# SeoYeonnLee/Video-Chapter-Generation

Hardware: AMD Instinct MI355X
Metric: clip-windows/sec (16f×224²+128tok) train-step at 1/2/4/8 MI355X; % HBM roofline (higher is better)
Workload: dtype bf16; 1 GPU; TwoStream train step: TSM-ResNet-50 + BERT-base + ChapterHead(mlp), B=64 windows/GPU of 16x224^2 frames + 128 tokens, fused clip+AdamW; global_batch=64, seq_len=128, frames=16, resolution=224, text_fill=n_valid ~ U[L/2, L], parallelism=dp1

## Files before the change

### video-chapter-generation_amd/csrc/igemm_fast.hip

```cpp
#include "fastload.h"

namespace vcg {

typedef __attribute__((address_space(3))) char lds_char;
__device__ __forceinline__ uint32_t lds_u32(const void* p) { return (uint32_t)(uintptr_t)(const lds_char*)p; }

template <int BN> __device__ __forceinline__ int st_slot(int row, int chunk) {
  if constexpr (BN == 128) return chunk ^ (row & 15);
  else return chunk ^ ((row >> 1) & 7);
}

template <int BM, int BN>
__device__ __forceinline__ void stage_put(bf16_t* stA, bf16_t* stB, int wm, int wn, int lane, int i, int j,
                                          const float (&v)[4]) {
  const int g = lane >> 4, ci = lane & 15;
  const int trow = (wm & 1) * 64 + i * 16 + ci;
  const int tcol = wn * (BN / 2) + j * 16 + 4 * g;
  bf16_t* reg = (BN == 128 && trow >= 64) ? stB : stA;
  const int row = BN == 128 ? (trow & 63) : trow;
  const uint32_t addr = lds_u32(reg + row * BN + 8 * st_slot<BN>(row, tcol >> 3) + (tcol & 7));
  uint2 q;
  q.x = (uint32_t)f2bf(v[0]) | ((uint32_t)f2bf(v[1]) << 16);
  q.y = (uint32_t)f2bf(v[2]) | ((uint32_t)f2bf(v[3]) << 16);
  asm volatile("ds_write_b64 %0, %1" ::"v"(addr), "v"(q) : "memory");
// ... 1161 lines not shown
    if (i < steps) issue_next(i);
  int kt = 0, tile = 0, cur = 0;
  for (int s = 0; s < steps; ++s) {
    const int ahead = min(STAGES - 1, steps - 1 - s);
    if (s + STAGES - 1 < steps) issue_next(cur == 0 ? STAGES - 1 : cur - 1);
    if (STAGES == 3 && ahead >= 2) __builtin_amdgcn_s_waitcnt(waitcnt_vm(2 * NLD));
    else if (ahead >= 1) __builtin_amdgcn_s_waitcnt(waitcnt_vm(NLD));
    else __builtin_amdgcn_s_waitcnt(waitcnt_vm(0));
    __builtin_amdgcn_s_barrier();
    if (kt == 0) FAST_STAMP(tile, 0);
    const bf16_t* Ac = As + cur * AE;
    const bf16_t* Bc = Bs + cur * BE;
#pragma unroll
    for (int s2 = 0; s2 < 2; ++s2) {
      s16x8 af[MT], bfr[NT];
#pragma unroll
      for (int i = 0; i < MT; ++i) af[i] = fast_frag(Ac, wm * 64 + i * 16, lane, s2);
#pragma unroll
      for (int j = 0; j < NT; ++j) bfr[j] = fast_frag(Bc, wn * (BN / 2) + j * 16, lane, s2);
#pragma unroll
      for (int i = 0; i < MT; ++i)
#pragma unroll
        for (int j = 0; j < NT; ++j)
          acc[i][j] = __builtin_amdgcn_mfma_f32_16x16x32_bf16(bfr[j], af[i], acc[i][j], 0, 0, 0);
    }
    __builtin_amdgcn_s_waitcnt(0xC07F);
    __builtin_amdgcn_s_barrier();
    if (++kt == ntiles) {
      FAST_STAMP(tile, 1);
      const int mt = by + tile * gy;
      bf16_t* stA = As + cur * AE;
      bf16_t* stB = BM == 256 ? stA + 64 * BN : Bs + cur * BE;
      const bool staged = true;
      if constexpr (BWD) {
#pragma unroll
        for (int h = 0; h < BM / 128; ++h) {
          if ((wm >> 1) == h) {
#pragma unroll
            for (int j = 0; j < NT; ++j)
#pragma unroll
              for (int i = 0; i < MT; ++i) {
                float v[4] = {acc[i][j][0], acc[i][j][1], acc[i][j][2], acc[i][j][3]};
                if constexpr (AM == OP_DENSE_K2) {
#pragma unroll
                  for (int r = 0; r < 4; ++r) v[r] += bv[j][r];
                }
                stage_put<BM, BN>(stA, stB, wm, wn, lane, i, j, v);
              }
          }
          FAST_STAMP(tile, 2);
          stage_flush_bwd<BM, BN, EPI == EPI_BWD_AFF>(stA, stB, p, Cout, mt * BM + 128 * h, n0, cpar, b1, b2, b3, p.M);
        }
      } else if constexpr (EPI == EPI_STATS) {
#pragma unroll
        for (int h = 0; h < BM / 128; ++h) {
          if ((wm >> 1) == h) {
#pragma unroll
            for (int j = 0; j < NT; ++j)
#pragma unroll
              for (int i = 0; i < MT; ++i) {
                float v[4] = {acc[i][j][0], acc[i][j][1], acc[i][j][2], acc[i][j][3]};
                stage_put<BM, BN>(stA, stB, wm, wn, lane, i, j, v);
              }
          }
          stage_flush_stats<BM, BN>(stA, stB, p, Cout, mt * BM + 128 * h, n0, scnt, b1, b2, b3, p.M);
        }
      } else if constexpr (EPI == EPI_STORE_AUX) {
        if constexpr (BM == 128) epilogue_staged_aux<BM, BN>(acc, p, bv, Cout, stA, stB, mt * BM, n0, wm, wn, lane);
      } else if (BM == 256 || (staged && !RES && p.aux == nullptr && (p.ldc & 7) == 0 &&
                               ((uintptr_t)p.C & 15) == 0)) {
        epilogue_staged<BM, BN>(acc, p, bv, Cout, stA, stB, mt * BM, n0, wm, wn, lane, p.M);
      } else if (RES && (staged || p.obits) && p.aux == nullptr &&
                 (RES == 2 ? (staged && !p.res_sc) : (p.res_round && p.act == ACT_RELU)) &&
                 ((p.ldc | p.ldr | p.N) & 7) == 0 && (((uintptr_t)p.residual | (uintptr_t)p.C) & 15) == 0) {
        if constexpr (BM == 128 && RES)
          epilogue_staged_res<BM, BN, RES == 2>(acc, p, bv, Cout, Res, stA, stB, mt * BM, n0, wm, wn, lane, p.M);
      } else {
        if constexpr (BM == 128)
          gemm_epilogue<bf16_t, BM, BN, EPI>(acc, p, red, bv, Cout, Res, mt * BM, n0, wm, wn, lane, mt, mtiles);
      }
      FAST_STAMP(tile, 3);
#pragma unroll
      for (int i = 0; i < MT; ++i)
#pragma unroll
        for (int j = 0; j < NT; ++j) acc[i][j] = f32x4{0.f, 0.f, 0.f, 0.f};
      kt = 0;
      ++tile;
    }
    cur = cur == STAGES - 1 ? 0 : cur + 1;
  }
  if constexpr (EPI == EPI_STATS)
    stats_finish<BM, BN>(p, reinterpret_cast<float*>(smem), scnt, b1, b2, b3, n0, by, bx, gy, (p.M + 127) / 128);
  if constexpr (BWD) {
    if (p.bwd.nred > 0) bwd_finish<BM, BN>(p, reinterpret_cast<float*>(smem), cpar + 4 * BN, b1, b2, b3, n0, by);
  }
}

template <int BM, int BN, int AM, int EPI, int RES, int XF = 0>
__global__ __launch_bounds__(BM * 2) __attribute__((amdgpu_waves_per_eu(EPI == EPI_BWD_AFF && BN == 64 ? 3 : 2)))
void igemm_fast_kernel(GemmParams p) {
  if constexpr (EPI == EPI_BWD_STREAM && BN == 128)
    bwd_stream128_body<XF>(p);
  else if constexpr (EPI == EPI_BWD_STREAM)
    bwd_stream_body<AM, XF>(p);
  else
    igemm_fast_body<BM, BN, AM, EPI, RES>(p);
}

static int grid_rows(int M, int N, int z, int BM, int BN, int epi) {
  const int nx = (N + BN - 1) / BN, mtiles = (M + BM - 1) / BM;
  const int resident = (BM == 256 ? 1 : (BN == 128 || epi == EPI_BWD ? 2 : 3)) * 256;
  int gy = resident / (nx * z);
  if (gy >= 8) gy &= ~7;
  if (gy > mtiles) gy = mtiles >= 8 ? (mtiles & ~7) : mtiles;
  if (gy < 1) gy = 1;
  return gy;
}

static int fast_bn_cols(int N) { return (N % 128 == 0 || N > 64 * 3) ? 128 : 64; }

static int fast_bm(int, int, int, bool) { return 128; }

int fast_grid_rows(int M, int N, int z, int epi) {
  return grid_rows(M, N, z, fast_bm(M, N, z, false), fast_bn_cols(N), epi);
}

static bool bwd_light(const GemmParams& p) {
  const BwdEpi& e = p.bwd;
  return !e.res && !e.bits && !e.y2 && e.tsm_T == 0;
}


constexpr int PATCH_MAXPIX = 256;
constexpr int PATCH_SLICES = PATCH_MAXPIX / 8;
constexpr int PATCH_RING = 3;

struct PatchGeom {
  int R, TM, TPI, PW, NP, NS;
  unsigned long long* stamps;
};
#define PATCH_STAMP(k)                                                                        \
  do {                                                                                        \
    if (g.stamps && blockIdx.x == 0 && threadIdx.x == 0 && lt < 64) g.stamps[lt * 6 + (k)] = __builtin_amdgcn_s_memtime(); \
  } while (0)

__device__ __forceinline__ int pswz(int pix, int c) { return (c + (pix & ~1)) & 7; }

__device__ __forceinline__ s16x8 patch_frag(const bf16_t* P, int pix, int lane, int s2) {
  return *reinterpret_cast<const s16x8*>(P + pix * 64 + 8 * pswz(pix, 4 * s2 + (lane >> 4)));
}

typedef __attribute__((address_space(3))) const char patch_lds_t;

template <int EPI, bool DG, int PW>
__global__ __launch_bounds__(256) __attribute__((amdgpu_waves_per_eu(1, 1)))
void conv3x3_patch_kernel(GemmParams p, PatchGeom g) {
  static_assert(PW == 32 || PW == 64, "patch row pitch");
  constexpr int BM = 128, BN = 64, NW = 4, MT = 4, NT = 2;
  constexpr int PE = PATCH_SLICES * 512;
  constexpr int YE = 128 * 64;
  constexpr bool BWD = EPI == EPI_BWD_AFF;
  constexpr int NY = BWD ? PATCH_RING : 0;
  constexpr int NIP = 8 + (BWD ? 4 : 0);
  __shared__ __attribute__((aligned(1024))) char smem[(PATCH_RING * PE + NY * YE) * 2];
  bf16_t* Ps = reinterpret_cast<bf16_t*>(smem);
  bf16_t* Ys = Ps + PATCH_RING * PE;

  const int tid = threadIdx.x, lane = tid & 63, wave = __builtin_amdgcn_readfirstlane(tid >> 6);
  const int wm = wave >> 1, wn = wave & 1;
  const int nx = p.N / BN, gy = gridDim.x / nx;
  int bx, by;
  if ((gy & 7) == 0) {
    const int sidx = blockIdx.x >> 3;
    bx = sidx % nx;
    by = (sidx / nx) * 8 + (blockIdx.x & 7);
  } else {
    bx = blockIdx.x % nx;
    by = blockIdx.x / nx;
  }
  const int n0 = bx * BN;
  bf16_t* Cout = reinterpret_cast<bf16_t*>(p.C);
  const int mtiles = p.M / g.TM;
  const int my_tiles = by < mtiles ? (mtiles - 1 - by) / gy + 1 : 0;
  const BwdEpi& e = p.bwd;
  if (my_tiles == 0) {
    if (BWD && e.nred > 0 && tid < BN)
      for (int r = 0; r < e.nred; ++r) e.part[((long long)by * e.nred + r) * p.N + n0 + tid] = 0.f;
    return;
  }

  const OpArgs& a = p.a;
  const uint32_t nbytes = (uint32_t)min(a.bytes, (long long)0xFFFFFF00LL);
  const __amdgpu_buffer_rsrc_t rsrc =
      __builtin_amdgcn_make_buffer_rsrc(const_cast<void*>(a.ptr), 0, nbytes, 0x00020000);
  const uint32_t ybytes = (BWD && e.y) ? (uint32_t)min((long long)p.M * p.ldc * 2, (long long)0xFFFFFF00LL) : 0u;
  const __amdgpu_buffer_rsrc_t yrsrc =
      __builtin_amdgcn_make_buffer_rsrc(const_cast<void*>(BWD ? e.y : a.ptr), 0, ybytes, 0x00020000);
  const int HW = a.H * a.W;
  auto issue_piece = [&](int lt, int tg, int img, int h0, int q) {
    if (q < 8) {
      bf16_t* dst = Ps + (lt % PATCH_RING) * PE;
      const int slice = min(wave + NW * q, g.NS - 1);
      const int pix = 8 * slice + (lane >> 3);
      const int pr = pix / PW, pc = pix % PW;
      const int h = h0 - 1 + pr, w = pc - 1;
      const bool ok = pix < g.NP && (unsigned)h < (unsigned)a.H && (unsigned)w < (unsigned)a.W;
      const int csrc = ((lane & 7) - (pix & ~1)) & 7;
      const uint32_t voff = ok ? (uint32_t)((((img * HW + h * a.W + w) << 6) + 8 * csrc) * 2) : nbytes;
      __builtin_amdgcn_raw_ptr_buffer_load_lds(rsrc, (lds_void_t*)(dst + slice * 512), 16, voff, 0, 0, 0);
    } else if constexpr (BWD) {
      bf16_t* ydst = Ys + (lt % PATCH_RING) * YE;
      const int r0 = 32 * wave + 8 * (q - 8), r = r0 + (lane >> 3);
      const uint32_t voff =
          r < g.TM ? (uint32_t)(((long long)(tg * g.TM + r) * p.ldc + n0 + 8 * (lane & 7)) * 2) : ybytes;
      __builtin_amdgcn_raw_ptr_buffer_load_lds(yrsrc, (lds_void_t*)(ydst + r0 * 64), 16, ybytes ? voff : 0u, 0, 0, 0);
    }
  };
  auto issue_tile = [&](int lt) {
    const int tg = by + lt * gy, img = tg / g.TPI, h0 = (tg - img * g.TPI) * g.R;
#pragma unroll
    for (int q = 0; q < NIP; ++q) issue_piece(lt, tg, img, h0, q);
  };
  int rowpix[MT];
#pragma unroll
  for (int i = 0; i < MT; ++i) {
    const int ml = wm * 64 + i * 16 + (lane & 15);
    const int r = ml / a.W, w = ml - r * a.W;
    rowpix[i] = ml < g.TM ? r * PW + w : 0;
  }
  s16x8 breg[9][2][NT];
  {
    const bf16_t* B = reinterpret_cast<const bf16_t*>(p.b.ptr);
#pragma unroll
    for (int j = 0; j < NT; ++j) {
      const bf16_t* row = B + (long long)(n0 + wn * (BN / 2) + j * 16 + (lane & 15)) * p.b.ld + 8 * (lane >> 4);
#pragma unroll
      for (int t = 0; t < 9; ++t)
#pragma unroll
        for (int s2 = 0; s2 < 2; ++s2) breg[t][s2][j] = *reinterpret_cast<const s16x8*>(row + 64 * t + 32 * s2);
    }
  }
  constexpr int CPR = BN / 8, KC = 128 * BN / 8 / 256;
  const int cc = tid % CPR, ncol = n0 + 8 * cc;
  float mu[8], sc[8], sh[8];
#pragma unroll
  for (int i = 0; i < 8; ++i) {
    mu[i] = (BWD && e.mean) ? e.mean[ncol + i] : 0.f;
    sc[i] = (BWD && e.msc) ? e.msc[ncol + i] : 0.f;
    sh[i] = (BWD && e.msh) ? e.msh[ncol + i] : 0.f;
  }
  __builtin_amdgcn_s_waitcnt(waitcnt_vm(0));
  issue_tile(0);
  if (my_tiles > 1) issue_tile(1);

  const bool mask = BWD && e.msc != nullptr && e.y != nullptr;
  float b1[8], b2[8], b3[8];
  int scnt = 0;
#pragma unroll
  for (int i = 0; i < 8; ++i) b1[i] = b2[i] = b3[i] = 0.f;
  uint4 q[KC], yq[KC];
  int pm0 = 0, pmlim = 0;
  auto process = [&](int k) {
    const int m = pm0 + (tid + 256 * k) / CPR;
    if (m >= pmlim) return;
    uint4* dst = reinterpret_cast<uint4*>(Cout + (long long)m * p.ldc + ncol);
    if constexpr (EPI == EPI_STORE) {
      *dst = q[k];
    } else if constexpr (EPI == EPI_STATS) {
      *dst = q[k];
      float v[8];
      unpack8(q[k], v);
      if (scnt == 0) {
#pragma unroll
        for (int i = 0; i < 8; ++i) b1[i] = v[i];
      }
      ++scnt;
#pragma unroll
      for (int i = 0; i < 8; ++i) {
        const float d = v[i] - b1[i];
        b2[i] += d;
        b3[i] = fmaf(d, d, b3[i]);
      }
    } else {
      float v[8], yy[8];
      unpack8(q[k], v);
      unpack8(yq[k], yy);
      if (mask) {
#pragma unroll
        for (int i = 0; i < 8; ++i) v[i] = fmaf(yy[i], sc[i], sh[i]) > 0.f ? v[i] : 0.f;
      }
      uint4 o;
      o.x = (uint32_t)f2bf(v[0]) | ((uint32_t)f2bf(v[1]) << 16);
      o.y = (uint32_t)f2bf(v[2]) | ((uint32_t)f2bf(v[3]) << 16);
      o.z = (uint32_t)f2bf(v[4]) | ((uint32_t)f2bf(v[5]) << 16);
      o.w = (uint32_t)f2bf(v[6]) | ((uint32_t)f2bf(v[7]) << 16);
      *dst = o;
      if (e.nred > 0) {
        unpack8(o, v);
#pragma unroll
        for (int i = 0; i < 8; ++i) {
          b1[i] += v[i];
          b2[i] = fmaf(v[i], yy[i] - mu[i], b2[i]);
        }
      }
    }
  };

  for (int lt = 0; lt < my_tiles; ++lt) {
    PATCH_STAMP(0);
    if (lt + 1 < my_tiles) __builtin_amdgcn_s_waitcnt(waitcnt_vm(NIP));
    else __builtin_amdgcn_s_waitcnt(waitcnt_vm(0));
    __builtin_amdgcn_s_barrier();
    PATCH_STAMP(1);
    const bool pre = lt + 2 < my_tiles;
    const int tg2 = by + (lt + 2) * gy, img2 = tg2 / g.TPI, h02 = (tg2 - img2 * g.TPI) * g.R;
    const bool prev = lt > 0;
    PATCH_STAMP(2);
    const bf16_t* P = Ps + (lt % PATCH_RING) * PE;
    f32x4 acc[MT][NT];
#pragma unroll
    for (int i = 0; i < MT; ++i)
#pragma unroll
      for (int j = 0; j < NT; ++j) acc[i][j] = f32x4{0.f, 0.f, 0.f, 0.f};
    uint32_t fa[MT][3][2];
#pragma unroll
    for (int i = 0; i < MT; ++i)
#pragma unroll
      for (int c = 0; c < 3; ++c) {
        const int pix = rowpix[i] + c;
        const uint32_t a0 = lds_u32(P + pix * 64 + 8 * pswz(pix, lane >> 4));
        fa[i][c][0] = a0;
        fa[i][c][1] = a0 ^ 64u;
      }
    auto unit_reads = [&](s16x8 (&f)[MT], int u) {
      const int t = u >> 1, kh = t / 3, kw = t - 3 * (t / 3);
      const int rh = DG ? 2 - kh : kh, cw = DG ? 2 - kw : kw;
#pragma unroll
      for (int i = 0; i < MT; ++i)
        f[i] = *reinterpret_cast<const __attribute__((address_space(3))) s16x8*>(
            (patch_lds_t*)(uintptr_t)fa[i][cw][u & 1] + rh * PW * 128);
    };
    s16x8 af[3][MT];
    unit_reads(af[0], 0);
    unit_reads(af[1], 1);
#pragma unroll
    for (int u = 0; u < 18; ++u) {
      if (u + 2 < 18) unit_reads(af[(u + 2) % 3], u + 2);
      if (u < NIP && pre) issue_piece(lt + 2, tg2, img2, h02, u);
      if constexpr (NIP + 2 * KC <= 18) {
        if (u >= NIP && ((u - NIP) & 1) == 0 && ((u - NIP) >> 1) < KC && prev) process((u - NIP) >> 1);
      } else {
        if (u >= 18 - KC && prev) process(u - (18 - KC));
      }
#pragma unroll
      for (int i = 0; i < MT; ++i)
#pragma unroll
        for (int j = 0; j < NT; ++j)
          acc[i][j] = __builtin_amdgcn_mfma_f32_16x16x32_bf16(breg[u >> 1][u & 1][j], af[u % 3][i], acc[i][j], 0, 0, 0);
      __builtin_amdgcn_sched_barrier(0);
    }
    PATCH_STAMP(3);
    __builtin_amdgcn_s_waitcnt(0xC07F);
    __builtin_amdgcn_s_barrier();
    PATCH_STAMP(4);
    bf16_t* stA = Ps + (lt % PATCH_RING) * PE;
#pragma unroll
    for (int j = 0; j < NT; ++j)
#pragma unroll
      for (int i = 0; i < MT; ++i) {
        float v[4] = {acc[i][j][0], acc[i][j][1], acc[i][j][2], acc[i][j][3]};
        stage_put<BM, BN>(stA, stA, wm, wn, lane, i, j, v);
      }
    asm volatile("s_waitcnt lgkmcnt(0)" ::: "memory");
    __builtin_amdgcn_s_barrier();
    const bf16_t* Y = Ys + (lt % PATCH_RING) * YE;
#pragma unroll
    for (int k = 0; k < KC; ++k) {
      const int trow = (tid + 256 * k) / CPR;
      asm volatile("ds_read_b128 %0, %1" : "=v"(q[k]) : "v"(lds_u32(stA + trow * BN + 8 * st_slot<BN>(trow, cc))) : "memory");
      if constexpr (BWD)
        asm volatile("ds_read_b128 %0, %1" : "=v"(yq[k]) : "v"(lds_u32(Y + trow * 64 + 8 * cc)) : "memory");
    }
    asm volatile("s_waitcnt lgkmcnt(0)" ::: "memory");
    pm0 = (by + lt * gy) * g.TM;
    pmlim = pm0 + g.TM;
    PATCH_STAMP(5);
  }
#pragma unroll
  for (int k = 0; k < KC; ++k) process(k);
  __builtin_amdgcn_s_waitcnt(waitcnt_vm(0));
  if constexpr (EPI == EPI_STATS)
    stats_finish<BM, BN>(p, reinterpret_cast<float*>(smem), scnt, b1, b2, b3, n0, by, bx, gy, (p.M + 127) / 128);
  if constexpr (BWD) {
    if (e.nred > 0) {
      float* inv = reinterpret_cast<float*>(smem) + 3 * 256 * 8;
      __syncthreads();
      if (tid < BN) inv[tid] = e.invstd ? e.invstd[n0 + tid] : 0.f;
      bwd_finish<BM, BN>(p, reinterpret_cast<float*>(smem), inv, b1, b2, b3, n0, by);
    }
  }
}

constexpr int SPATCH_MAXPIX = 1024;

struct StemGeom {
  int R, TM, TPI, PW, NP, NS, NR;
  unsigned long long* stamps;
};

template <int EPI>
__global__ __launch_bounds__(256) __attribute__((amdgpu_waves_per_eu(2, 2)))
void stem_patch_kernel(GemmParams p, StemGeom g) {
  constexpr int BM = 128, BN = 64, NW = 4, MT = 4, NT = 2, KHMAX = 8, RING = 3, NIP = 4;
  constexpr int PE = SPATCH_MAXPIX * 8;
  __shared__ __attribute__((aligned(1024))) char smem[RING * PE * 2];
  bf16_t* Ps = reinterpret_cast<bf16_t*>(smem);
  const int tid = threadIdx.x, lane = tid & 63, wave = __builtin_amdgcn_readfirstlane(tid >> 6);
  const int wm = wave >> 1, wn = wave & 1;
  const int nx = p.N / BN, gy = gridDim.x / nx;
  int bx, by;
  if ((gy & 7) == 0) {
    const int sidx = blockIdx.x >> 3;
    bx = sidx % nx;
    by = (sidx / nx) * 8 + (blockIdx.x & 7);
  } else {
    bx = blockIdx.x % nx;
    by = blockIdx.x / nx;
  }
  const int n0 = bx * BN;
  bf16_t* Cout = reinterpret_cast<bf16_t*>(p.C);
  const int mtiles = p.M / g.TM;
  const int my_tiles = by < mtiles ? (mtiles - 1 - by) / gy + 1 : 0;
  if (my_tiles == 0) return;

  const OpArgs& a = p.a;
  const int KH = a.KH;
  const uint32_t nbytes = (uint32_t)min(a.bytes, (long long)0xFFFFFF00LL);
  const __amdgpu_buffer_rsrc_t rsrc =
      __builtin_amdgcn_make_buffer_rsrc(const_cast<void*>(a.ptr), 0, nbytes, 0x00020000);
  auto issue_piece = [&](int lt, int img, int h0, int q) {
    bf16_t* dst = Ps + (lt % RING) * PE;
    const int slice = min(wave + NW * q, g.NS - 1);
    const int pix = 64 * slice + lane;
    const int pr = pix / g.PW, pc = pix - pr * g.PW;
    const int ih = 2 * h0 - a.pad + pr, sx = pc - a.pw;
    const bool ok = pix < g.NP && (unsigned)ih < (unsigned)a.H && (unsigned)sx < (unsigned)a.W;
    const uint32_t voff = ok ? (uint32_t)((((img * a.H + ih) * a.W + sx) << 3) * 2) : nbytes;
    __builtin_amdgcn_raw_ptr_buffer_load_lds(rsrc, (lds_void_t*)(dst + slice * 512), 16, voff, 0, 0, 0);
  };
  auto issue_tile = [&](int lt) {
    const int tg = by + lt * gy, img = tg / g.TPI, h0 = (tg - img * g.TPI) * g.R;
#pragma unroll
    for (int q = 0; q < NIP; ++q) issue_piece(lt, img, h0, q);
  };
  int rowpix[MT];
#pragma unroll
  for (int i = 0; i < MT; ++i) {
    const int ml = wm * 64 + i * 16 + (lane & 15);
    const int r = ml / a.GW, w = ml - r * a.GW;
    rowpix[i] = ml < g.TM ? 2 * r * g.PW + w : 0;
  }
  s16x8 breg[KHMAX][NT];
  {
    const bf16_t* B = reinterpret_cast<const bf16_t*>(p.b.ptr);
#pragma unroll
    for (int j = 0; j < NT; ++j) {
      const bf16_t* row = B + (long long)(n0 + wn * (BN / 2) + j * 16 + (lane & 15)) * p.b.ld + 8 * (lane >> 4);
#pragma unroll
      for (int kh = 0; kh < KHMAX; ++kh)
        breg[kh][j] = kh < KH ? *reinterpret_cast<const s16x8*>(row + 32 * kh) : s16x8{0, 0, 0, 0, 0, 0, 0, 0};
    }
  }
  constexpr int CPR = BN / 8, KC = 128 * BN / 8 / 256;
  const int cc = tid % CPR, ncol = n0 + 8 * cc;
  __builtin_amdgcn_s_waitcnt(waitcnt_vm(0));
  issue_tile(0);
  if (my_tiles > 1) issue_tile(1);

  float b1[8], b2[8], b3[8];
  int scnt = 0;
#pragma unroll
  for (int i = 0; i < 8; ++i) b1[i] = b2[i] = b3[i] = 0.f;
  uint4 q[KC];
  int pm0 = 0, pmlim = 0;
  auto process = [&](int k) {
    const int m = pm0 + (tid + 256 * k) / CPR;
    if (m >= pmlim) return;
    *reinterpret_cast<uint4*>(Cout + (long long)m * p.ldc + ncol) = q[k];
    if constexpr (EPI == EPI_STATS) {
      float v[8];
      unpack8(q[k], v);
      if (scnt == 0) {
#pragma unroll
        for (int i = 0; i < 8; ++i) b1[i] = v[i];
      }
      ++scnt;
#pragma unroll
      for (int i = 0; i < 8; ++i) {
        const float d = v[i] - b1[i];
        b2[i] += d;
        b3[i] = fmaf(d, d, b3[i]);
      }
    }
  };

  for (int lt = 0; lt < my_tiles; ++lt) {
    if (lt + 1 < my_tiles) __builtin_amdgcn_s_waitcnt(waitcnt_vm(NIP));
    else __builtin_amdgcn_s_waitcnt(waitcnt_vm(0));
    __builtin_amdgcn_s_barrier();
    const bool pre = lt + 2 < my_tiles;
    const int tg2 = by + (lt + 2) * gy, img2 = tg2 / g.TPI, h02 = (tg2 - img2 * g.TPI) * g.R;
    const bool prev = lt > 0;
    const bf16_t* P = Ps + (lt % RING) * PE;
#pragma unroll
    for (int i = 0; i < MT; ++i) asm volatile("" : "+v"(rowpix[i]));
    f32x4 acc[MT][NT];
#pragma unroll
    for (int i = 0; i < MT; ++i)
#pragma unroll
      for (int j = 0; j < NT; ++j) acc[i][j] = f32x4{0.f, 0.f, 0.f, 0.f};
    auto unit_reads = [&](s16x8 (&f)[MT], int kh) {
#pragma unroll
      for (int i = 0; i < MT; ++i)
        f[i] = *reinterpret_cast<const s16x8*>(P + (rowpix[i] + kh * g.PW + (lane >> 4)) * 8);
    };
    s16x8 af[3][MT];
    unit_reads(af[0], 0);
    unit_reads(af[1], 1);
#pragma unroll
    for (int u = 0; u < KHMAX; ++u) {
      if (u < KH) {
        if (u + 2 < KH) unit_reads(af[(u + 2) % 3], u + 2);
        if (u < NIP && pre) issue_piece(lt + 2, img2, h02, u);
        if (u >= 1 && u - 1 < KC && prev) process(u - 1);
#pragma unroll
        for (int i = 0; i < MT; ++i)
#pragma unroll
          for (int j = 0; j < NT; ++j)
            acc[i][j] = __builtin_amdgcn_mfma_f32_16x16x32_bf16(breg[u][j], af[u % 3][i], acc[i][j], 0, 0, 0);
        __builtin_amdgcn_sched_barrier(0);
      }
    }
    if (prev) {
// ... 49 lines not shown
  g.PW = p.a.GW + p.a.KW - 1;
  g.NR = 2 * R + p.a.KH - 2;
  g.NP = g.NR * g.PW;
  g.NS = (g.NP + 63) / 64;
  return g;
}

static int patch_pitch(int W) { return W + 2 <= 32 ? 32 : 64; }

static int patch_rows(const GemmParams& p, int amode) {
  const char* e = getenv("VCG_NO_PATCH");
  const bool off = e && e[0] == '1';
  const OpArgs& a = p.a;
  if (off || (amode != OP_IM2COL && amode != OP_DGRAD) || a.C != 64 || a.KH != 3 || a.KW != 3 || a.stride != 1 ||
      a.pad != 1 || a.tsm_fold != 0 || a.tKW != 0 || a.sw != 0 || a.GH != a.H || a.GW != a.W || p.N % 64 != 0 ||
      p.K != 9 * 64 || p.batch_inner > 0 || p.residual || p.aux || p.bias || p.act != ACT_NONE || a.W + 2 > 64 ||
      !bwd_light(p) || p.bwd.nred > 2)
    return 0;
  for (int R = min(a.H, 128 / a.W); R >= 1; --R)
    if (a.H % R == 0 && (R + 2) * patch_pitch(a.W) <= PATCH_MAXPIX) return R;
  return 0;
}

static PatchGeom patch_geom(const GemmParams& p, int R) {
  PatchGeom g{};
  g.R = R;
  g.TM = R * p.a.W;
  g.TPI = p.a.H / R;
  g.PW = patch_pitch(p.a.W);
  g.NP = (R + 2) * g.PW;
  g.NS = (g.NP + 7) / 8;
  return g;
}

static int patch_grid_rows(const GemmParams& p, const PatchGeom& g) {
  const int nx = p.N / 64, mtiles = p.M / g.TM;
  int gy = 256 / nx;
  gy = min(gy, min(mtiles, (p.M + 127) / 128));
  if (gy >= 8) gy &= ~7;
  return max(gy, 1);
}

static bool bwd_stream_ok(const GemmParams& p) {
  const char* v = getenv("VCG_BWD_STREAM");
  if (v && v[0] == '0') return false;
  const BwdEpi& e = p.bwd;
  const bool dense = p.a.KH == 0 && p.a.GH == 0;
  if (!dense || (p.K != 64 && p.K != 128 && p.K != 256) || p.N % 64 != 0 || p.batch_inner > 0 || p.ldc != p.N || p.a.ld != p.K ||
      !e.res || e.msc || e.sub || bwd_light(p))
    return false;
  if ((e.y && !e.bits) || (e.y2 && !e.y)) return false;
  if ((e.y || e.bits) && e.nred < 2) return false;
  if (e.tsm_T > 0 && e.tsm_fold % 32 != 0) return false;
  if (p.K == 256 && ((e.tsm_T > 0 && e.tsm_fold % 64 != 0) || e.y)) return false;
  if (p.K == 256 && ((uintptr_t)p.b.ptr & 15 || p.b.ld % 8 != 0)) return false;
  if (((uintptr_t)p.C | (uintptr_t)e.res | (uintptr_t)e.y | (uintptr_t)e.y2 | (uintptr_t)p.a.ptr) & 15) return false;
  if (e.res_s > 1 && (p.M % e.hw) != 0) return false;
  if (e.pj > 0) {
    if (e.y || !e.bits || e.pj != 64 || p.K > 128 || ((uintptr_t)e.a2 & 15) || !e.ppart) return false;
    if (((uintptr_t)p.b.ptr & 15) || p.b.ld % 8 != 0) return false;
  }
  return true;
}

static int bwd_stream_tn(const GemmParams& p) {
  const BwdEpi& e = p.bwd;
  const char* v = getenv("VCG_BWD_STREAM");
  if ((v && v[0] == '6') || p.bwd.pj > 0) return 64;
  return p.K == 256 && p.N % 128 == 0 && !e.y && (e.tsm_T <= 0 || e.tsm_fold % 128 == 0) ? 128 : 64;
}

static int bwd_stream_rows(const GemmParams& p) {
  const int nx = p.N / bwd_stream_tn(p), mtiles = (p.M + 63) / 64;
  int gy = 256 / nx;
  if (gy >= 8) gy &= ~7;
  if (gy > mtiles) gy = mtiles >= 8 ? (mtiles & ~7) : mtiles;
  return gy < 1 ? 1 : gy;
}

bool fast_bwd_streams(const GemmParams& p) { return bwd_stream_ok(p); }

int fast_bwd_slots(const GemmParams& p) {
  if (bwd_stream_ok(p)) return bwd_stream_rows(p);
  const int R = patch_rows(p, OP_DGRAD);
  if (R > 0) return patch_grid_rows(p, patch_geom(p, R));
  return fast_grid_rows(p.M, p.N, 1, bwd_light(p) ? EPI_BWD_AFF : EPI_BWD);
}

template <int AM, int EPI, int RES>
static double algorithmic_bytes(const GemmParams& p, int z) {
  const double mn = (double)p.M * p.N * z;
  double b = (AM == OP_DENSE_K || AM == OP_DENSE_K2 ? 2.0 * p.M * (double)p.K * z : (double)p.a.bytes) + 2.0 * p.N * (double)p.K * z;
  b += 2.0 * mn;
  if (RES) b += 2.0 * mn;
  if (p.aux) b += 2.0 * mn;
  if constexpr (EPI == EPI_BWD || EPI == EPI_BWD_AFF) {
    const BwdEpi& e = p.bwd;
    if (e.res) b += 2.0 * mn / (e.res_s > 1 ? 4.0 : 1.0);
    if (e.y) b += 2.0 * mn;
    if (e.y2) b += 2.0 * mn;
    if (e.bits) b += mn / 8.0;
  }
  return b;
}

template <int BM, int BN, int AM, int EPI, int RES>
static int launch_fast(const GemmParams& p, int z, hipStream_t s) {
  const int nx = (p.N + BN - 1) / BN;
  const int gy = grid_rows(p.M, p.N, z, BM, BN, EPI);
  dim3 grid(nx * gy, 1, z);
  const int tk = timing_begin(s);
  hipLaunchKernelGGL((igemm_fast_kernel<BM, BN, AM, EPI, RES>), grid, dim3(BM * 2), 0, s, p);
  if (census_on()) { char t_[96]; snprintf(t_, sizeof(t_), "igemm_fast %dx%d a%d e%d r%d z%d", BM, BN, AM, EPI, RES, z); census_add(t_, p.M, p.N, p.K); }
  timing_end(tk, s, TIMING_FAST_GEMM, 2.0 * p.M * p.N * (double)p.K * z, algorithmic_bytes<AM, EPI, RES>(p, z));
  VCG_LAUNCH_CHECK();
  return VCG_OK;
}

template <int KC, int XF, int TN = 64>
static int launch_bwd_stream(const GemmParams& p, hipStream_t s) {
  const int nx = p.N / TN, gy = bwd_stream_rows(p);
  const int tk = timing_begin(s);
  hipLaunchKernelGGL((igemm_fast_kernel<256, TN, KC, EPI_BWD_STREAM, false, XF>), dim3(nx * gy), dim3(512), 0, s, p);
  if (census_on()) { char t_[96]; snprintf(t_, sizeof(t_), "igemm_fast_stream tn%d xf%d", TN, XF); census_add(t_, p.M, p.N, p.K); }
  const double pj = bwd_stream_pj(XF);
  timing_end(tk, s, TIMING_FAST_GEMM, 2.0 * p.M * p.N * (double)p.K + 2.0 * p.M * p.N * pj,
             algorithmic_bytes<OP_DENSE_K, EPI_BWD, false>(p, 1) + 2.0 * p.M * pj + 4.0 * p.N * pj);
  VCG_LAUNCH_CHECK();
  return VCG_OK;
}

template <int KC>
static int run_bwd_stream(const GemmParams& p, hipStream_t s) {
  if constexpr (KC == 4) {
    if (bwd_stream_tn(p) == 128)
      return p.bwd.bits ? launch_bwd_stream<4, XF_BITS, 128>(p, s) : launch_bwd_stream<4, 0, 128>(p, s);
  }
  if constexpr (KC <= 2) {
    if (p.bwd.pj == 64) return launch_bwd_stream<KC, XF_BITS | XF_P64>(p, s);
  }
  if (!p.bwd.y) return p.bwd.bits ? launch_bwd_stream<KC, XF_BITS>(p, s) : launch_bwd_stream<KC, 0>(p, s);
  if (!p.bwd.y2) return launch_bwd_stream<KC, XF_HASY>(p, s);
  return launch_bwd_stream<KC, XF_HASY | XF_Y2>(p, s);
}

template <int AM, int EPI, int RES = 0>
static int fast_bn(const GemmParams& p, int z, hipStream_t s) {
  if (fast_bn_cols(p.N) == 128) return launch_fast<128, 128, AM, EPI, RES>(p, z, s);
  return launch_fast<128, 64, AM, EPI, RES>(p, z, s);
}

static unsigned long long* g_patch_stamps = nullptr;

template <int EPI, bool DG, int PW>
static int launch_patch(const GemmParams& p, int R, hipStream_t s) {
  const PatchGeom g = patch_geom(p, R);
  const int gy = patch_grid_rows(p, g);
  const int tk = timing_begin(s);
  PatchGeom gs = g;
  const char* st = getenv("VCG_PATCH_STAMPS");
  if (st && st[0] == '1') {
    if (!g_patch_stamps && hipMalloc(&g_patch_stamps, 64 * 6 * 8) != hipSuccess) g_patch_stamps = nullptr;
    gs.stamps = g_patch_stamps;
  }
  hipLaunchKernelGGL((conv3x3_patch_kernel<EPI, DG, PW>), dim3((p.N / 64) * gy), dim3(256), 0, s, p, gs);
  if (census_on()) { char t_[96]; snprintf(t_, sizeof(t_), "conv3x3_patch e%d dg%d pw%d", EPI, (int)DG, PW); census_add(t_, p.M, p.N, p.K); }
  timing_end(tk, s, TIMING_PATCH_CONV, 2.0 * p.M * p.N * (double)p.K, algorithmic_bytes<OP_IM2COL, EPI, false>(p, 1));
  VCG_LAUNCH_CHECK();
  return VCG_OK;
}

template <int EPI>
static int launch_stem(const GemmParams& p, int R, hipStream_t s) {
  const StemGeom g = stem_geom(p, R);
  const int nx = p.N / 64, mtiles = p.M / g.TM;
  int gy = min((2 * 256) / nx, min(mtiles, (p.M + 127) / 128));
  if (gy >= 8) gy &= ~7;
  gy = max(gy, 1);
  const int tk = timing_begin(s);
  hipLaunchKernelGGL((stem_patch_kernel<EPI>), dim3(nx * gy), dim3(256), 0, s, p, g);
  if (census_on()) { char t_[96]; snprintf(t_, sizeof(t_), "stem_patch e%d", EPI); census_add(t_, p.M, p.N, p.K); }
  timing_end(tk, s, TIMING_PATCH_CONV, 2.0 * p.M * p.N * (double)p.K, algorithmic_bytes<OP_IM2COL, EPI, false>(p, 1));
  VCG_LAUNCH_CHECK();
  return VCG_OK;
}

int run_fast_gemm(GemmParams& p, int amode, int epi, int z, hipStream_t s) {
  if (p.a.ptr2) {
    if (amode != OP_DENSE_K || epi != EPI_BWD || z != 1 || !bwd_light(p) || p.a.split2 % FBK != 0) return -1;
    return fast_bn<OP_DENSE_K2, EPI_BWD_AFF>(p, z, s);
  }
  if (amode == OP_IM2COL && p.a.tsm_fold > 0) amode = OP_IM2COL_TSM;
  if (amode == OP_IM2COL && p.a.C < FBK) amode = OP_IM2COL_SMALLC;
  if (amode == OP_IM2COL_TSM && p.a.C < FBK) return -1;
  if (amode == OP_DGRAD && p.a.C < FBK) return -1;
  if (z == 1 && amode == OP_IM2COL_SMALLC && (epi == EPI_STATS || epi == EPI_STORE)) {
    const int R = stem_rows(p);
    if (R > 0) return epi == EPI_STATS ? launch_stem<EPI_STATS>(p, R, s) : launch_stem<EPI_STORE>(p, R, s);
  }
  if (z == 1) {
    const int R = patch_rows(p, amode);
    if (R > 0) {
      const bool w64 = patch_pitch(p.a.W) == 64;
      if (amode == OP_DGRAD) {
        if (epi == EPI_BWD)
          return w64 ? launch_patch<EPI_BWD_AFF, true, 64>(p, R, s) : launch_patch<EPI_BWD_AFF, true, 32>(p, R, s);
        if (epi == EPI_STATS)
          return w64 ? launch_patch<EPI_STATS, true, 64>(p, R, s) : launch_patch<EPI_STATS, true, 32>(p, R, s);
        if (epi == EPI_STORE)
          return w64 ? launch_patch<EPI_STORE, true, 64>(p, R, s) : launch_patch<EPI_STORE, true, 32>(p, R, s);
      } else {
        if (epi == EPI_STATS)
          return w64 ? launch_patch<EPI_STATS, false, 64>(p, R, s) : launch_patch<EPI_STATS, false, 32>(p, R, s);
        if (epi == EPI_STORE)
          return w64 ? launch_patch<EPI_STORE, false, 64>(p, R, s) : launch_patch<EPI_STORE, false, 32>(p, R, s);
      }
    }
  }
  if (amode != OP_IM2COL_SMALLC && gemm256_ok(p, amode, epi, z)) return run_gemm256(p, amode, epi, s);
  if (epi == EPI_BWD && amode == OP_DENSE_K && z == 1 && bwd_stream_ok(p))
    return p.K == 64 ? run_bwd_stream<1>(p, s) : p.K == 128 ? run_bwd_stream<2>(p, s) : run_bwd_stream<4>(p, s);
  if (epi == EPI_BWD && bwd_light(p)) {
    if (amode == OP_DGRAD) return fast_bn<OP_DGRAD, EPI_BWD_AFF>(p, z, s);
    if (amode == OP_DENSE_K) return fast_bn<OP_DENSE_K, EPI_BWD_AFF>(p, z, s);
    return -1;
  }
  if (epi == EPI_BWD) {
    if (amode == OP_DGRAD) return fast_bn<OP_DGRAD, EPI_BWD>(p, z, s);
    if (amode == OP_DENSE_K) return fast_bn<OP_DENSE_K, EPI_BWD>(p, z, s);
    return -1;
  }
  if (epi == EPI_STATS) {
    if (amode == OP_IM2COL_SMALLC) return fast_bn<OP_IM2COL_SMALLC, EPI_STATS>(p, z, s);
    if (amode == OP_IM2COL_TSM) return fast_bn<OP_IM2COL_TSM, EPI_STATS>(p, z, s);
    if (amode == OP_IM2COL) return fast_bn<OP_IM2COL, EPI_STATS>(p, z, s);
    if (amode == OP_DGRAD) return fast_bn<OP_DGRAD, EPI_STATS>(p, z, s);
    return fast_bn<OP_DENSE_K, EPI_STATS>(p, z, s);
  }
  if (p.residual) return p.act == ACT_GELU_BWD ? fast_bn<OP_DENSE_K, EPI_STORE, 2>(p, z, s)
                                               : fast_bn<OP_DENSE_K, EPI_STORE, 1>(p, z, s);
  if (p.aux && amode == OP_DENSE_K && (p.ldc & 7) == 0)
    return fast_bn<OP_DENSE_K, EPI_STORE_AUX>(p, z, s);
  if (amode == OP_IM2COL_SMALLC) return fast_bn<OP_IM2COL_SMALLC, EPI_STORE>(p, z, s);
  if (amode == OP_IM2COL_TSM) return fast_bn<OP_IM2COL_TSM, EPI_STORE>(p, z, s);
  if (amode == OP_IM2COL) return fast_bn<OP_IM2COL, EPI_STORE>(p, z, s);
  if (amode == OP_DGRAD) return fast_bn<OP_DGRAD, EPI_STORE>(p, z, s);
  return fast_bn<OP_DENSE_K, EPI_STORE>(p, z, s);
}

}

VCG_API int vcg_fast_stamps(unsigned long long* out, int n) {
#ifdef VCG_FAST_STAMPS
  n = n < 64 * 4 ? n : 64 * 4;
  return hipMemcpyFromSymbol(out, HIP_SYMBOL(vcg::g_fast_stamps), (size_t)n * 8, 0, hipMemcpyDeviceToHost) == hipSuccess
             ? 0 : 2;
#else
  (void)out;
  (void)n;
  return 1;
#endif
}

VCG_API int vcg_patch_stamps(unsigned long long* out, int n) {
  if (!vcg::g_patch_stamps) return 1;
  n = n < 64 * 6 ? n : 64 * 6;
  return hipMemcpy(out, vcg::g_patch_stamps, (size_t)n * 8, hipMemcpyDeviceToHost) == hipSuccess ? 0 : 2;
}
```

Measured before the change: 916.0 clip-windows/sec.

## Interleave patch conv epilogue and LDS reads at MFMA granularity

Restructures the 3x3 patch conv main loop so fragment reads, tile prefetch and the previous tile's epilogue are spread across individual MFMA issue slots rather than done per unit. The epilogue becomes a micro-stepped state machine using buffer stores with bounds-limited resources, and the mask check is made a compile-time template flag. Fragment LDS addresses are computed once and advanced per ring slot, and prefetch address arithmetic is simplified to avoid divides. The B fragments are pinned to AGPRs. The aim is to hide epilogue and load-issue latency under MFMA work, at the cost of much more complex scheduling code and higher register pressure.

```diff
diff --git a/video-chapter-generation_amd/csrc/igemm_fast.hip b/video-chapter-generation_amd/csrc/igemm_fast.hip
--- a/video-chapter-generation_amd/csrc/igemm_fast.hip
+++ b/video-chapter-generation_amd/csrc/igemm_fast.hip
@@ -1337,7 +1337,7 @@
 
 typedef __attribute__((address_space(3))) const char patch_lds_t;
 
-template <int EPI, bool DG, int PW>
+template <int EPI, bool DG, int PW, bool MASK = false>
 __global__ __launch_bounds__(256) __attribute__((amdgpu_waves_per_eu(1, 1)))
 void conv3x3_patch_kernel(GemmParams p, PatchGeom g) {
   static_assert(PW == 32 || PW == 64, "patch row pitch");
@@ -1382,23 +1382,29 @@
   const __amdgpu_buffer_rsrc_t yrsrc =
       __builtin_amdgcn_make_buffer_rsrc(const_cast<void*>(BWD ? e.y : a.ptr), 0, ybytes, 0x00020000);
   const int HW = a.H * a.W;
+  const int l8 = lane >> 3;
+  const uint32_t plane = (uint32_t)(l8 * 128 + 16 * (((lane & 7) - (l8 & ~1)) & 7));
+  const uint32_t ylane = (uint32_t)((l8 * p.ldc + 8 * (lane & 7)) * 2);
   auto issue_piece = [&](int lt, int tg, int img, int h0, int q) {
+    const bool live = tg < mtiles;
     if (q < 8) {
       bf16_t* dst = Ps + (lt % PATCH_RING) * PE;
-      const int slice = min(wave + NW * q, g.NS - 1);
-      const int pix = 8 * slice + (lane >> 3);
-      const int pr = pix / PW, pc = pix % PW;
-      const int h = h0 - 1 + pr, w = pc - 1;
-      const bool ok = pix < g.NP && (unsigned)h < (unsigned)a.H && (unsigned)w < (unsigned)a.W;
-      const int csrc = ((lane & 7) - (pix & ~1)) & 7;
-      const uint32_t voff = ok ? (uint32_t)((((img * HW + h * a.W + w) << 6) + 8 * csrc) * 2) : nbytes;
+      constexpr int SPR = PW / 8;
+      const int slice = wave + NW * q;
+      const int pr = (NW * q) / SPR, pc0 = 8 * ((NW * q) % SPR + wave);
+      const int hmax = live ? min(a.H, h0 + g.R + 1) : 0;
+      const int wlim = (unsigned)(h0 - 1 + pr) < (unsigned)hmax ? a.W : 0;
+      const uint32_t tbase = (uint32_t)((img * HW + (h0 - 1) * a.W - 1) * 128);
+      const uint32_t sbase = tbase + (uint32_t)((pr * a.W + pc0) * 128);
+      const uint32_t voff = (unsigned)(pc0 - 1 + l8) < (unsigned)wlim ? sbase + plane : nbytes;
       __builtin_amdgcn_raw_ptr_buffer_load_lds(rsrc, (lds_void_t*)(dst + slice * 512), 16, voff, 0, 0, 0);
     } else if constexpr (BWD) {
       bf16_t* ydst = Ys + (lt % PATCH_RING) * YE;
-      const int r0 = 32 * wave + 8 * (q - 8), r = r0 + (lane >> 3);
-      const uint32_t voff =
-          r < g.TM ? (uint32_t)(((long long)(tg * g.TM + r) * p.ldc + n0 + 8 * (lane & 7)) * 2) : ybytes;
-      __builtin_amdgcn_raw_ptr_buffer_load_lds(yrsrc, (lds_void_t*)(ydst + r0 * 64), 16, ybytes ? voff : 0u, 0, 0, 0);
+      const int r0 = 32 * wave + 8 * (q - 8);
+      const int rlim = (live && ybytes) ? g.TM - r0 : 0;
+      const uint32_t ytile = (uint32_t)(((long long)tg * g.TM * p.ldc + n0) * 2);
+      const uint32_t voff = l8 < rlim ? ytile + (uint32_t)(r0 * p.ldc * 2) + ylane : ybytes;
+      __builtin_amdgcn_raw_ptr_buffer_load_lds(yrsrc, (lds_void_t*)(ydst + r0 * 64), 16, voff, 0, 0, 0);
     }
   };
   auto issue_tile = [&](int lt) {
@@ -1426,6 +1432,8 @@
     }
   }
   constexpr int CPR = BN / 8, KC = 128 * BN / 8 / 256;
+  constexpr int NST = KC;
+  static_assert(4 * KC <= 18, "one epilogue slice per unit");
   const int cc = tid % CPR, ncol = n0 + 8 * cc;
   float mu[8], sc[8], sh[8];
 #pragma unroll
@@ -1435,115 +1443,170 @@
     sh[i] = (BWD && e.msh) ? e.msh[ncol + i] : 0.f;
   }
   __builtin_amdgcn_s_waitcnt(waitcnt_vm(0));
+#pragma unroll
+  for (int t = 0; t < 9; ++t)
+#pragma unroll
+    for (int s2 = 0; s2 < 2; ++s2)
+#pragma unroll
+      for (int j = 0; j < NT; ++j) asm volatile("" : "+a"(breg[t][s2][j]));
+  uint32_t fa[MT][3][2];
+#pragma unroll
+  for (int i = 0; i < MT; ++i)
+#pragma unroll
+    for (int c = 0; c < 3; ++c) {
+      const int pix = rowpix[i] + c;
+      const uint32_t a0 = lds_u32(Ps + pix * 64 + 8 * pswz(pix, lane >> 4));
+      fa[i][c][0] = a0;
+      fa[i][c][1] = a0 ^ 64u;
+    }
   issue_tile(0);
-  if (my_tiles > 1) issue_tile(1);
-
-  const bool mask = BWD && e.msc != nullptr && e.y != nullptr;
+  issue_tile(1);
+
   float b1[8], b2[8], b3[8];
-  int scnt = 0;
 #pragma unroll
   for (int i = 0; i < 8; ++i) b1[i] = b2[i] = b3[i] = 0.f;
-  uint4 q[KC], yq[KC];
-  int pm0 = 0, pmlim = 0;
-  auto process = [&](int k) {
-    const int m = pm0 + (tid + 256 * k) / CPR;
-    if (m >= pmlim) return;
-    uint4* dst = reinterpret_cast<uint4*>(Cout + (long long)m * p.ldc + ncol);
+  pk_u32x4 qw[KC], yw[KC];
+  uint32_t ow[4];
+#pragma unroll
+  for (int k = 0; k < KC; ++k) qw[k] = yw[k] = pk_u32x4{0u, 0u, 0u, 0u};
+  const int trow0 = tid / CPR;
+  const uint32_t ovoff = (uint32_t)((trow0 * p.ldc + ncol) * 2), ovstep = (uint32_t)(32 * p.ldc * 2);
+  const uint32_t obytes = (uint32_t)(g.TM * p.ldc * 2);
+  auto out_rsrc = [&](long long m0, uint32_t bytes) {
+    return __builtin_amdgcn_make_buffer_rsrc(Cout + m0 * p.ldc, 0, bytes, 0x00020000);
+  };
+  __amdgpu_buffer_rsrc_t orsrc = out_rsrc(0, 0u);
+  int plim = 0;
+  bool pfirst = true;
+#define PATCH_PIN(x) asm volatile("" : "+v"(x))
+  float ev0 = 0.f, ev1 = 0.f, ey0 = 0.f, ey1 = 0.f, es0 = 0.f, es1 = 0.f;
+  uint32_t eo = 0u, ew = 0u, ewy = 0u;
+  bool ec0 = false, ec1 = false;
+  auto epi_gap = [&](int k, int h, int m) {
+    const bool valid = trow0 + 32 * k < plim;
     if constexpr (EPI == EPI_STORE) {
-      *dst = q[k];
+      if (h == 0 && m == 3) __builtin_amdgcn_raw_buffer_store_b128(qw[k], orsrc, ovoff + k * ovstep, 0, 0);
     } else if constexpr (EPI == EPI_STATS) {
-      *dst = q[k];
-      float v[8];
-      unpack8(q[k], v);
-      if (scnt == 0) {
-#pragma unroll
-        for (int i = 0; i < 8; ++i) b1[i] = v[i];
-      }
-      ++scnt;
-#pragma unroll
-      for (int i = 0; i < 8; ++i) {
-        const float d = v[i] - b1[i];
-        b2[i] += d;
-        b3[i] = fmaf(d, d, b3[i]);
+      float &s0 = b1[2 * h], &s1 = b1[2 * h + 1];
+      if (m == 0) {
+        ev0 = __uint_as_float(qw[k][h] << 16);
+        ev1 = __uint_as_float(qw[k][h] & 0xffff0000u);
+        PATCH_PIN(ev0); PATCH_PIN(ev1);
+      } else if (m == 1 && k == 0) {
+        const bool init = valid & pfirst;
+        s0 = init ? ev0 : s0;
+        s1 = init ? ev1 : s1;
+        PATCH_PIN(s0); PATCH_PIN(s1);
+      } else if (m == 3) {
+        if (h == 3) __builtin_amdgcn_raw_buffer_store_b128(qw[k], orsrc, ovoff + k * ovstep, 0, 0);
+        ev0 -= s0;
+        ev1 -= s1;
+        PATCH_PIN(ev0); PATCH_PIN(ev1);
+      } else if (m == 4) {
+        ev0 = valid ? ev0 : 0.f;
+        ev1 = valid ? ev1 : 0.f;
+        PATCH_PIN(ev0); PATCH_PIN(ev1);
+      } else if (m == 5) {
+        b2[2 * h] += ev0;
+        b2[2 * h + 1] += ev1;
+        PATCH_PIN(b2[2 * h]); PATCH_PIN(b2[2 * h + 1]);
+      } else if (m == 6) {
+        b3[2 * h] = fmaf(ev0, ev0, b3[2 * h]);
+        b3[2 * h + 1] = fmaf(ev1, ev1, b3[2 * h + 1]);
+        PATCH_PIN(b3[2 * h]); PATCH_PIN(b3[2 * h + 1]);
       }
     } else {
-      float v[8], yy[8];
-      unpack8(q[k], v);
-      unpack8(yq[k], yy);
-      if (mask) {
-#pragma unroll
-        for (int i = 0; i < 8; ++i) v[i] = fmaf(yy[i], sc[i], sh[i]) > 0.f ? v[i] : 0.f;
-      }
-      uint4 o;
-      o.x = (uint32_t)f2bf(v[0]) | ((uint32_t)f2bf(v[1]) << 16);
-      o.y = (uint32_t)f2bf(v[2]) | ((uint32_t)f2bf(v[3]) << 16);
-      o.z = (uint32_t)f2bf(v[4]) | ((uint32_t)f2bf(v[5]) << 16);
-      o.w = (uint32_t)f2bf(v[6]) | ((uint32_t)f2bf(v[7]) << 16);
-      *dst = o;
-      if (e.nred > 0) {
-        unpack8(o, v);
-#pragma unroll
-        for (int i = 0; i < 8; ++i) {
-          b1[i] += v[i];
-          b2[i] = fmaf(v[i], yy[i] - mu[i], b2[i]);
-        }
+      if (m == 0) {
+        ew = qw[k][h], ewy = yw[k][h];
+        PATCH_PIN(ew); PATCH_PIN(ewy);
+        ev0 = __uint_as_float(ew << 16);
+        ey0 = __uint_as_float(ewy << 16);
+        PATCH_PIN(ev0); PATCH_PIN(ey0);
+      } else if (m == 1) {
+        ev1 = __uint_as_float(ew & 0xffff0000u);
+        ey1 = __uint_as_float(ewy & 0xffff0000u);
+        PATCH_PIN(ev1); PATCH_PIN(ey1);
+      } else if (m == 3) {
+        ec0 = fmaf(ey0, sc[2 * h], sh[2 * h]) > 0.f;
+        ec1 = fmaf(ey1, sc[2 * h + 1], sh[2 * h + 1]) > 0.f;
+      } else if (m == 4) {
+        if constexpr (MASK) ev0 = ec0 ? ev0 : 0.f;
+        if constexpr (MASK) ev1 = ec1 ? ev1 : 0.f;
+        asm("v_cvt_pk_bf16_f32 %0, %1, %2" : "=v"(eo) : "v"(ev0), "v"(ev1));
+        eo = valid ? eo : 0u;
+        PATCH_PIN(eo);
+      } else if (m == 5) {
+        ow[h] = eo;
+        if (h == 3)
+          __builtin_amdgcn_raw_buffer_store_b128(pk_u32x4{ow[0], ow[1], ow[2], ow[3]}, orsrc, ovoff + k * ovstep,
+                                                 0, 0);
+        ev0 = __uint_as_float(eo << 16);
+        ev1 = __uint_as_float(eo & 0xffff0000u);
+        es0 = ey0 - mu[2 * h];
+        PATCH_PIN(ev0); PATCH_PIN(ev1); PATCH_PIN(es0);
+      } else if (m == 6) {
+        es1 = ey1 - mu[2 * h + 1];
+        b1[2 * h] += ev0;
+        b2[2 * h] = fmaf(ev0, es0, b2[2 * h]);
+        PATCH_PIN(es1); PATCH_PIN(b1[2 * h]); PATCH_PIN(b2[2 * h]);
+      } else if (m == 7) {
+        b1[2 * h + 1] += ev1;
+        b2[2 * h + 1] = fmaf(ev1, es1, b2[2 * h + 1]);
+        PATCH_PIN(b1[2 * h + 1]); PATCH_PIN(b2[2 * h + 1]);
       }
     }
   };
+  constexpr int U0 = 18 - 4 * KC;
 
   for (int lt = 0; lt < my_tiles; ++lt) {
     PATCH_STAMP(0);
-    if (lt + 1 < my_tiles) __builtin_amdgcn_s_waitcnt(waitcnt_vm(NIP));
-    else __builtin_amdgcn_s_waitcnt(waitcnt_vm(0));
+    if (lt == 0) __builtin_amdgcn_s_waitcnt(waitcnt_vm(NIP));
+    else __builtin_amdgcn_s_waitcnt(waitcnt_vm(NIP + NST));
     __builtin_amdgcn_s_barrier();
     PATCH_STAMP(1);
-    const bool pre = lt + 2 < my_tiles;
     const int tg2 = by + (lt + 2) * gy, img2 = tg2 / g.TPI, h02 = (tg2 - img2 * g.TPI) * g.R;
-    const bool prev = lt > 0;
     PATCH_STAMP(2);
-    const bf16_t* P = Ps + (lt % PATCH_RING) * PE;
     f32x4 acc[MT][NT];
 #pragma unroll
     for (int i = 0; i < MT; ++i)
 #pragma unroll
       for (int j = 0; j < NT; ++j) acc[i][j] = f32x4{0.f, 0.f, 0.f, 0.f};
-    uint32_t fa[MT][3][2];
-#pragma unroll
-    for (int i = 0; i < MT; ++i)
-#pragma unroll
-      for (int c = 0; c < 3; ++c) {
-        const int pix = rowpix[i] + c;
-        const uint32_t a0 = lds_u32(P + pix * 64 + 8 * pswz(pix, lane >> 4));
-        fa[i][c][0] = a0;
-        fa[i][c][1] = a0 ^ 64u;
-      }
-    auto unit_reads = [&](s16x8 (&f)[MT], int u) {
+    auto frag_read = [&](s16x8& f, int u, int i) {
       const int t = u >> 1, kh = t / 3, kw = t - 3 * (t / 3);
       const int rh = DG ? 2 - kh : kh, cw = DG ? 2 - kw : kw;
-#pragma unroll
-      for (int i = 0; i < MT; ++i)
-        f[i] = *reinterpret_cast<const __attribute__((address_space(3))) s16x8*>(
-            (patch_lds_t*)(uintptr_t)fa[i][cw][u & 1] + rh * PW * 128);
+      f = *reinterpret_cast<const __attribute__((address_space(3))) s16x8*>(
+          (patch_lds_t*)(uintptr_t)fa[i][cw][u & 1] + rh * PW * 128);
     };
     s16x8 af[3][MT];
-    unit_reads(af[0], 0);
-    unit_reads(af[1], 1);
+#pragma unroll
+    for (int i = 0; i < MT; ++i) frag_read(af[0][i], 0, i);
+#pragma unroll
+    for (int i = 0; i < MT; ++i) frag_read(af[1][i], 1, i);
+    constexpr int LGKM4 = 0xC47F, LGKM0 = 0xC07F;
+    __builtin_amdgcn_s_waitcnt(LGKM4);
+    __builtin_amdgcn_sched_barrier(0);
 #pragma unroll
     for (int u = 0; u < 18; ++u) {
-      if (u + 2 < 18) unit_reads(af[(u + 2) % 3], u + 2);
-      if (u < NIP && pre) issue_piece(lt + 2, tg2, img2, h02, u);
-      if constexpr (NIP + 2 * KC <= 18) {
-        if (u >= NIP && ((u - NIP) & 1) == 0 && ((u - NIP) >> 1) < KC && prev) process((u - NIP) >> 1);
-      } else {
-        if (u >= 18 - KC && prev) process(u - (18 - KC));
-      }
-#pragma unroll
-      for (int i = 0; i < MT; ++i)
-#pragma unroll
-        for (int j = 0; j < NT; ++j)
-          acc[i][j] = __builtin_amdgcn_mfma_f32_16x16x32_bf16(breg[u >> 1][u & 1][j], af[u % 3][i], acc[i][j], 0, 0, 0);
-      __builtin_amdgcn_sched_barrier(0);
-    }
+#pragma unroll
+      for (int m = 0; m < MT * NT; ++m) {
+        const int i = m / NT, j = m % NT;
+        acc[i][j] = __builtin_amdgcn_mfma_f32_16x16x32_bf16(breg[u >> 1][u & 1][j], af[u % 3][i], acc[i][j], 0, 0, 0);
+        if (m < 2 && u + 2 < 18) {
+          frag_read(af[(u + 2) % 3][2 * m], u + 2, 2 * m);
+          frag_read(af[(u + 2) % 3][2 * m + 1], u + 2, 2 * m + 1);
+        }
+        if (m == 2 && u < NIP) issue_piece(lt + 2, tg2, img2, h02, u);
+        if (u >= U0) epi_gap((u - U0) >> 2, (u - U0) & 3, m);
+        if (m == MT * NT - 1 && u + 2 < 18) __builtin_amdgcn_s_waitcnt(LGKM4);
+        if (m == MT * NT - 1 && u + 2 == 18) __builtin_amdgcn_s_waitcnt(LGKM0);
+        __builtin_amdgcn_sched_barrier(0);
+      }
+    }
+    const uint32_t fstep = (lt + 1) % PATCH_RING == 0 ? (uint32_t)(-(PATCH_RING - 1) * PE * 2) : (uint32_t)(PE * 2);
+#pragma unroll
+    for (int i = 0; i < MT; ++i)
+#pragma unroll
+      for (int c = 0; c < 3; ++c) fa[i][c][0] += fstep, fa[i][c][1] += fstep;
     PATCH_STAMP(3);
     __builtin_amdgcn_s_waitcnt(0xC07F);
     __builtin_amdgcn_s_barrier();
@@ -1562,18 +1625,23 @@
 #pragma unroll
     for (int k = 0; k < KC; ++k) {
       const int trow = (tid + 256 * k) / CPR;
-      asm volatile("ds_read_b128 %0, %1" : "=v"(q[k]) : "v"(lds_u32(stA + trow * BN + 8 * st_slot<BN>(trow, cc))) : "memory");
+      asm volatile("ds_read_b128 %0, %1" : "=v"(qw[k]) : "v"(lds_u32(stA + trow * BN + 8 * st_slot<BN>(trow, cc))) : "memory");
       if constexpr (BWD)
-        asm volatile("ds_read_b128 %0, %1" : "=v"(yq[k]) : "v"(lds_u32(Y + trow * 64 + 8 * cc)) : "memory");
+        asm volatile("ds_read_b128 %0, %1" : "=v"(yw[k]) : "v"(lds_u32(Y + trow * 64 + 8 * cc)) : "memory");
     }
     asm volatile("s_waitcnt lgkmcnt(0)" ::: "memory");
-    pm0 = (by + lt * gy) * g.TM;
-    pmlim = pm0 + g.TM;
+    orsrc = out_rsrc((long long)(by + lt * gy) * g.TM, obytes);
+    plim = g.TM;
+    pfirst = lt == 0;
     PATCH_STAMP(5);
   }
 #pragma unroll
-  for (int k = 0; k < KC; ++k) process(k);
+  for (int s = 0; s < 4 * KC; ++s)
+#pragma unroll
+    for (int m = 0; m < 8; ++m) epi_gap(s >> 2, s & 3, m);
+#undef PATCH_PIN
   __builtin_amdgcn_s_waitcnt(waitcnt_vm(0));
+  const int scnt = my_tiles * max(0, min(KC, (g.TM - trow0 + 31) / 32));
   if constexpr (EPI == EPI_STATS)
     stats_finish<BM, BN>(p, reinterpret_cast<float*>(smem), scnt, b1, b2, b3, n0, by, bx, gy, (p.M + 127) / 128);
   if constexpr (BWD) {
@@ -1929,7 +1997,7 @@
 
 static unsigned long long* g_patch_stamps = nullptr;
 
-template <int EPI, bool DG, int PW>
+template <int EPI, bool DG, int PW, bool MASK = false>
 static int launch_patch(const GemmParams& p, int R, hipStream_t s) {
   const PatchGeom g = patch_geom(p, R);
   const int gy = patch_grid_rows(p, g);
@@ -1940,7 +2008,7 @@
     if (!g_patch_stamps && hipMalloc(&g_patch_stamps, 64 * 6 * 8) != hipSuccess) g_patch_stamps = nullptr;
     gs.stamps = g_patch_stamps;
   }
-  hipLaunchKernelGGL((conv3x3_patch_kernel<EPI, DG, PW>), dim3((p.N / 64) * gy), dim3(256), 0, s, p, gs);
+  hipLaunchKernelGGL((conv3x3_patch_kernel<EPI, DG, PW, MASK>), dim3((p.N / 64) * gy), dim3(256), 0, s, p, gs);
   if (census_on()) { char t_[96]; snprintf(t_, sizeof(t_), "conv3x3_patch e%d dg%d pw%d", EPI, (int)DG, PW); census_add(t_, p.M, p.N, p.K); }
   timing_end(tk, s, TIMING_PATCH_CONV, 2.0 * p.M * p.N * (double)p.K, algorithmic_bytes<OP_IM2COL, EPI, false>(p, 1));
   VCG_LAUNCH_CHECK();
@@ -1980,8 +2048,12 @@
     if (R > 0) {
       const bool w64 = patch_pitch(p.a.W) == 64;
       if (amode == OP_DGRAD) {
-        if (epi == EPI_BWD)
+        if (epi == EPI_BWD) {
+          if (p.bwd.msc != nullptr && p.bwd.y != nullptr)
+            return w64 ? launch_patch<EPI_BWD_AFF, true, 64, true>(p, R, s)
+                       : launch_patch<EPI_BWD_AFF, true, 32, true>(p, R, s);
           return w64 ? launch_patch<EPI_BWD_AFF, true, 64>(p, R, s) : launch_patch<EPI_BWD_AFF, true, 32>(p, R, s);
+        }
         if (epi == EPI_STATS)
           return w64 ? launch_patch<EPI_STATS, true, 64>(p, R, s) : launch_patch<EPI_STATS, true, 32>(p, R, s);
         if (epi == EPI_STORE)
```

After: 923.0 clip-windows/sec (median of 6 runs). No clear change (+0.8%).
